# blasif/cocons

Hardware: AMD Instinct MI355X
Metric: -2loglik evals/sec (dense cov_rns + Cholesky/solve/log-det, fp64) at n=10000 (higher is better)
Workload: dtype f64

## Files before the change

cocons_amd/csrc/chol.hip:

```cpp
#include <hip/hip_runtime.h>
#include <limits.h>
#include <stdlib.h>
#include <string.h>
#include <algorithm>
#include <atomic>
#include <vector>
#include "kernels.h"

namespace cocons {

typedef double d4 __attribute__((ext_vector_type(4)));

#define MFMA64(a, b, c) __builtin_amdgcn_mfma_f64_16x16x4f64((a), (b), (c), 0, 0, 0)
#define MFMA64_NEGA(a, b, c) __builtin_amdgcn_mfma_f64_16x16x4f64((a), (b), (c), 0, 0, 1)
#define LDS_T __attribute__((address_space(3)))

__device__ __forceinline__ void blk_mma(d4 &acc, const d4 &P, const d4 &Q)
{
    acc = MFMA64(Q[0], P[0], acc);
    acc = MFMA64(Q[1], P[1], acc);
    acc = MFMA64(Q[2], P[2], acc);
    acc = MFMA64(Q[3], P[3], acc);
}

// ... 1356 lines not shown

#pragma unroll
        for (int v = 0; v < RPT / 2; ++v) {
            stI[v] = *(const d2 *)(gI + 2 * v);
            stJ[v] = *(const d2 *)(gJ + 2 * v);
        }
#pragma unroll
        for (int v = 0; v < RPT / 2; ++v) {
            *(d2 *)(&sI[0][kc * LDT + rg + 2 * v]) = stI[v];
            *(d2 *)(&sJ[0][kc * LDT + rg + 2 * v]) = stJ[v];
        }
        __syncthreads();

        for (int ch = 0; ch < nch; ++ch) {
            const int cur = ch & 1;
            if (ch + 1 < nch) {
                const double *pI = gI + (size_t)(ch + 1) * KC * a.ldp;
                const double *pJ = gJ + (size_t)(ch + 1) * KC * a.ldp;
#pragma unroll
                for (int v = 0; v < RPT / 2; ++v) {
                    stI[v] = *(const d2 *)(pI + 2 * v);
                    stJ[v] = *(const d2 *)(pJ + 2 * v);
                }
            }
            const double *bI = &sI[cur][ro + (TM / 2) * wi];
            const double *bJ = &sJ[cur][ro + (TM / WY) * wj];
#pragma unroll
            for (int s = 0; s < KC / 4; ++s) {
                double pi_[NB], pj_[NBY];
#pragma unroll
                for (int x = 0; x < NB; ++x) pi_[x] = bI[s * 4 * LDT + 16 * x];
#pragma unroll
                for (int y = 0; y < NBY; ++y) pj_[y] = bJ[s * 4 * LDT + 16 * y];
#pragma unroll
                for (int x = 0; x < NB; ++x)
#pragma unroll
                    for (int y = 0; y < NBY; ++y) acc[x][y] = MFMA64(pj_[y], pi_[x], acc[x][y]);
            }
            if (ch + 1 < nch) {
#pragma unroll
                for (int v = 0; v < RPT / 2; ++v) {
                    *(d2 *)(&sI[cur ^ 1][kc * LDT + rg + 2 * v]) = stI[v];
                    *(d2 *)(&sJ[cur ^ 1][kc * LDT + rg + 2 * v]) = stJ[v];
                }
            }
            __syncthreads();
        }
        unsigned Lnext = 0;
        if (a.queue && t2 == 0)
            Lnext = gridDim.x + __hip_atomic_fetch_add(a.queue, 1u, __ATOMIC_RELAXED, __HIP_MEMORY_SCOPE_AGENT);
        unsigned cve = cvo;
        asm volatile("" : "+v"(cve));
#pragma unroll
        for (int x = 0; x < NB; ++x)
#pragma unroll
            for (int y = 0; y < NBY; ++y) {
                d4 cv;
#pragma unroll
                for (int r = 0; r < 4; ++r) {
                    const double *cp = (const double *)((const char *)(Cb + 16 * x) + (cve + (unsigned)(16 * y + 4 * r) * ldcb));
                    cv[r] = a.c_wt ? load_wt(cp) : *cp;
                }
                cv -= acc[x][y];
                if (wt_wg) {
#pragma unroll
                    for (int r = 0; r < 4; ++r)
                        store_wt((double *)((char *)(Cb + 16 * x) + (cve + (unsigned)(16 * y + 4 * r) * ldcb)), cv[r]);
                } else {
#pragma unroll
                    for (int r = 0; r < 4; ++r)
                        *(double *)((char *)(Cb + 16 * x) + (cve + (unsigned)(16 * y + 4 * r) * ldcb)) = cv[r];
                }
            }
        if (wt_wg) {
            asm volatile("s_waitcnt vmcnt(0)" ::: "memory");
            __syncthreads();
            if (t2 == 0 && sig_wg) signal_add(a.sig + a.sig_tile + sig_Ti);
        }
        if (!a.queue) break;
        if (t2 == 0) *share = Lnext;
        __syncthreads();
        L = (unsigned)__builtin_amdgcn_readfirstlane((int)*share);
        if (L >= a.ntiles) break;
    }
}

struct DagStep {
    unsigned base;
    unsigned near;
    unsigned tpos, nT;
    int H, W;
    int tj0;
    int k0, K;
    int nstrip, two;
    int need;
    int nd_next;
    int split;
    unsigned p2, p3;
};

struct DagArgs {
    double *A; size_t lda;
    double *P;
    const double *Wt;
    const DagStep *steps; int nsteps;
    unsigned ntasks;
    unsigned *queue;
    unsigned *tdone;
    unsigned *pdone; int pstride;
    unsigned *pall;
    double *partbuf;
    unsigned *dcount;
    unsigned *sig;
    unsigned *out, *xr;
    unsigned *abort_word;
    const unsigned *alive;
    unsigned xcc_quota;
    unsigned *hw;
    unsigned long long *trace;
    const unsigned *ftab;
    unsigned xcd_g;
    unsigned *xcnt;
};

constexpr unsigned DAG_XCD_LAG = 64u;
__device__ __forceinline__ unsigned dag_position(unsigned c, unsigned cls, unsigned g)
{
    return ((c >> g) << (g + 3u)) | (cls << g) | (c & ((1u << g) - 1u));
}

__device__ __forceinline__ bool dag_wait(const DagArgs &a, unsigned *word, unsigned need, unsigned code, unsigned L)
{
    const unsigned long long t0 = __builtin_amdgcn_s_memrealtime();
    for (unsigned it = 0;; ++it) {
        const unsigned v = poll_word(word, it);
        if (v >= need) break;
        if (__hip_atomic_load(a.abort_word, __ATOMIC_RELAXED, __HIP_MEMORY_SCOPE_AGENT) != 0u) return false;
        if (it > (unsigned)(ENGINE_TIMEOUT_TICKS / 100ull) ||
            ((it & 1023u) == 1023u && __builtin_amdgcn_s_memrealtime() - t0 > WALL_BACKSTOP_TICKS)) {
            if (__hip_atomic_exchange(a.abort_word, code, __ATOMIC_RELAXED, __HIP_MEMORY_SCOPE_AGENT) == 0u) {
                unsigned *d = a.queue + 8;
                d[0] = L; d[1] = code; d[2] = (unsigned)(word - a.queue); d[3] = need; d[4] = v;
                d[5] = (unsigned)(__builtin_amdgcn_s_memrealtime() - t0);
                d[6] = it;
            }
            return false;
        }
        __builtin_amdgcn_s_sleep(16);
    }
    __builtin_amdgcn_fence(__ATOMIC_ACQUIRE, "wavefront");
    return true;
}

__global__ void __launch_bounds__(256, 8)
dag_kernel(DagArgs a)
{
    constexpr int TM = 64, KC = 4, RING = 4, STG = 2 * KC * TM;
    __shared__ double smem[RING * STG + 2];
    unsigned *share = (unsigned *)&smem[RING * STG];
    const int tid = threadIdx.x;
    const int wave_s = __builtin_amdgcn_readfirstlane(tid >> 6);
    const DagStep *__restrict__ steps = a.steps;
    const unsigned ldab = 8u * (unsigned)a.lda;
    int known = 0;
    const unsigned myx = (hw_where() >> 28) & 7u;
    const bool loyal = ((blockIdx.x >> 3) & 1u) == 0u;
    if (tid == 0) {
        bool take = true;
        if (a.xcc_quota) {
            const unsigned c = __hip_atomic_load(a.alive + 16 + myx, __ATOMIC_RELAXED, __HIP_MEMORY_SCOPE_AGENT);
            if (c) {
                const unsigned less = 7u * (c - 1u);
                const unsigned quota = a.xcc_quota > less + 8u ? a.xcc_quota - less : 8u;
                take = __hip_atomic_fetch_add(a.queue + 16 + myx, 1u, __ATOMIC_RELAXED, __HIP_MEMORY_SCOPE_AGENT) < quota;
            }
        }
        unsigned first = 0xffffffffu;
        if (take) {
            if (a.xcd_g) first = dag_position(__hip_atomic_fetch_add(a.xcnt + 32u * myx, 1u, __ATOMIC_RELAXED, __HIP_MEMORY_SCOPE_AGENT), myx, a.xcd_g);
            else first = __hip_atomic_fetch_add(a.queue, 1u, __ATOMIC_RELAXED, __HIP_MEMORY_SCOPE_AGENT);
        }
        share[1] = first;
        share[2] = 0u;
    }
    __syncthreads();
    unsigned L = (unsigned)__builtin_amdgcn_readfirstlane((int)share[1]);
    __syncthreads();
    if (L >= a.ntasks) return;
    for (;;) {
        int lo = 0, hi = a.nsteps - 1;
        while (lo < hi) {
            const int mid = (lo + hi + 1) >> 1;
            if (steps[mid].base <= L) lo = mid; else hi = mid - 1;
        }
        const int s = lo;
        const DagStep st = steps[s];
        const unsigned q = L - st.base;
        if (a.trace && tid == 0) {
            a.trace[4 * (size_t)L] = __builtin_amdgcn_s_memrealtime();
            if (a.hw) a.hw[2 * (size_t)L] = hw_where();
        }
        const int t = st.tj0 >> 1;
        const unsigned per_u = 2u * (unsigned)st.nstrip, nA = per_u + (unsigned)st.nd_next, perBC = st.two ? per_u : 0u;
        int tkind = -1;
        unsigned tu = 0, qt_u = q;
        if (q >= st.tpos) {
            if (q < st.tpos + nA) { tu = q - st.tpos; tkind = tu < per_u ? 0 : 3; }
            else if (q < st.p2) qt_u = q - nA;
            else if (q < st.p2 + perBC) { tu = q - st.p2; tkind = 1; }
            else if (q < st.p3) qt_u = q - nA - perBC;
            else if (q < st.p3 + perBC) { tu = q - st.p3; tkind = 2; }
            else qt_u = q - nA - 2u * perBC;
        }
        const bool isT = tkind >= 0;
        const double *gIb, *gJb;
        unsigned ldib, ldjb, ldob = ldab;
        int K, i_wt = 0, store_only = 0, strip_task = 0;
        double *Cb;
        const double *pa = nullptr;
        unsigned *w0 = nullptr, *w1 = nullptr, *w2 = nullptr, *we = nullptr, *we2 = nullptr, *dn;
        unsigned n0 = 0, n1 = 0, n2 = 0, ne = 0, dval = 0;
        int sigT = -1;
        int prio = 0;
        if (!isT) {
            const int qt = (int)qt_u;
            int ti, tj;
            if (a.ftab && qt >= (int)st.near) {
                const unsigned e = a.ftab[a.ftab[s] + (unsigned)(qt - (int)st.near)];
                tj = st.tj0 + (int)(e & 0xffffu); ti = st.tj0 + (int)(e >> 16);
            } else {
                int jl = 0, jh = st.W - 1;
                while (jl < jh) {
                    const int mid = (jl + jh + 1) >> 1;
                    if (mid * st.H - mid * (mid - 1) / 2 <= qt) jl = mid; else jh = mid - 1;
                }
                tj = st.tj0 + jl; ti = tj + (qt - (jl * st.H - jl * (jl - 1) / 2));
            }
            const double *Ps = s == 0 ? a.A : a.P;
            gIb = Ps + (size_t)ti * TM + (size_t)st.k0 * a.lda;
            gJb = Ps + (size_t)tj * TM + (size_t)st.k0 * a.lda;
            ldib = ldab; ldjb = ldab; K = st.K;
            Cb = a.A + (size_t)ti * TM + (size_t)tj * TM * a.lda;
            if (s > known) {
                w0 = a.pall + s; n0 = (unsigned)st.H;
                w1 = a.pdone + (size_t)s * a.pstride + (ti - st.tj0); n1 = (unsigned)st.need;
                w2 = a.pdone + (size_t)s * a.pstride + (tj - st.tj0); n2 = (unsigned)st.need;
            }
            we = a.tdone + (ti * (ti + 1) / 2 + tj); ne = (unsigned)s;
            dn = we; dval = (unsigned)s + 1u;
            const int Ti = (ti >> 1) - t, Tj = (tj >> 1) - t;
            if (Ti >= 0 && Ti <= st.two && Tj >= 0 && Tj <= Ti) {
                sigT = t + Ti; prio = 3;
                if (st.split) {
                    const int ta = ti - st.tj0, tb = tj - st.tj0, dd = ta * (ta + 1) / 2 + tb;
                    gIb += (size_t)TILE * a.lda; gJb += (size_t)TILE * a.lda; K = TILE;
                    pa = a.partbuf + ((size_t)(s & 1) * 16 + dd) * (TM * TM);
                    we2 = a.dcount + (size_t)s * 16 + dd;
                }
            }
        } else {
            const int per = 2 * st.nstrip;
            const size_t c_t = (size_t)t * TILE, c_t1 = c_t + TILE;
            prio = 2;
            const int stage = tkind;
            int strip = 0, h = 0, row64 = 0;
            if (stage != 3) {
                strip = (int)(tu >> 1); h = (int)(tu & 1u);
                row64 = st.tj0 + (st.two ? 4 : 2) + strip;
                strip_task = 1;
            }
            dn = a.pdone + (size_t)(s + 1) * a.pstride + strip;
            if (stage == 3) {
                const int dd = (int)tu - per;
                const int ta = c_tri_ib[dd], tb = dd - ta * (ta + 1) / 2;
                const int tj0n = st.tj0 + 4;
                const size_t k0n = (size_t)(s + 1) * 2 * TILE;
                gIb = a.P + (size_t)(tj0n + ta) * TM + k0n * a.lda; ldib = ldab;
                gJb = a.P + (size_t)(tj0n + tb) * TM + k0n * a.lda; ldjb = ldab;
                K = TILE;
                Cb = a.partbuf + ((size_t)((s + 1) & 1) * 16 + dd) * (TM * TM); store_only = 1; ldob = 8u * TM;
                w0 = a.pdone + (size_t)(s + 1) * a.pstride + ta; n0 = 2u;
                w1 = a.pdone + (size_t)(s + 1) * a.pstride + tb; n1 = 2u;
                dn = a.dcount + (size_t)(s + 1) * 16 + dd;
            } else if (stage == 0) {
                gIb = a.A + (size_t)row64 * TM + c_t * a.lda; ldib = ldab; i_wt = 1;
                gJb = a.Wt + (size_t)t * TILE * TILE + TM * h; ldjb = 8u * TILE;
                K = TM * (h + 1);
                Cb = a.P + (size_t)row64 * TM + (c_t + TM * h) * a.lda; store_only = 1;
                w0 = a.out + t; n0 = 1u;
                w1 = a.tdone + (row64 * (row64 + 1) / 2 + 2 * t); n1 = (unsigned)s + 1u;
                w2 = w1 + 1; n2 = n1;
            } else if (stage == 1) {
                gIb = a.P + (size_t)row64 * TM + c_t * a.lda; ldib = ldab;
                gJb = a.P + (c_t1 + TM * h) + c_t * a.lda; ldjb = ldab;
                K = TILE;
                Cb = a.A + (size_t)row64 * TM + (c_t1 + TM * h) * a.lda;
                w0 = dn; n0 = 2u;
                w1 = a.xr + t; n1 = 1u;
                we = a.tdone + (row64 * (row64 + 1) / 2 + 2 * (t + 1) + h); ne = (unsigned)s + 1u;
            } else {
                gIb = a.A + (size_t)row64 * TM + c_t1 * a.lda; ldib = ldab; i_wt = 1;
                gJb = a.Wt + (size_t)(t + 1) * TILE * TILE + TM * h; ldjb = 8u * TILE;
                K = TM * (h + 1);
                Cb = a.P + (size_t)row64 * TM + (c_t1 + TM * h) * a.lda; store_only = 1;
                w0 = dn; n0 = 4u;
                w1 = a.out + t + 1; n1 = 1u;
            }
        }
        if (prio == 3) __builtin_amdgcn_s_setprio(3);
        else if (prio == 2) __builtin_amdgcn_s_setprio(2);
        else __builtin_amdgcn_s_setprio(0);

        if (w0) {
            if (tid == 0) {
                unsigned ok;
                if (!isT) {
                    if (__hip_atomic_load(w0, __ATOMIC_RELAXED, __HIP_MEMORY_SCOPE_AGENT) >= n0) ok = 2u;
                    else ok = (dag_wait(a, w1, n1, abort_code(0xb00u, (unsigned)s), L) &&
                               dag_wait(a, w2, n2, abort_code(0xc00u, (unsigned)s), L)) ? 1u : 0u;
                } else {
                    bool o = dag_wait(a, w0, n0, abort_code(0xa00u, (unsigned)s), L);
                    if (o && w1) o = dag_wait(a, w1, n1, abort_code(0xb00u, (unsigned)s), L);
                    if (o && w2) o = dag_wait(a, w2, n2, abort_code(0xc00u, (unsigned)s), L);
                    ok = o ? 1u : 0u;
                }
                *share = ok;
            }
            asm volatile("s_waitcnt vmcnt(0)" ::: "memory");
            __syncthreads();
            const unsigned ok = (unsigned)__builtin_amdgcn_readfirstlane((int)*share);
            __syncthreads();
            if (!ok) return;
            if (ok == 2u) known = s;
        }

        if (a.trace && tid == 0) a.trace[4 * (size_t)L + 1] = __builtin_amdgcn_s_memrealtime();
        int lane;
        asm volatile("v_mbcnt_lo_u32_b32 %0, -1, 0\n\tv_mbcnt_hi_u32_b32 %0, -1, %0" : "=v"(lane));
        const int wave = wave_s, t2 = 64 * wave + lane;
        const int wi = wave & 1, wj = wave >> 1;
        const bool opJ = wave >= 2;
        const char *gsrc = opJ ? (const char *)gJb : (const char *)gIb;
        const unsigned ldg = opJ ? ldjb : ldib, cstep = (unsigned)KC * ldg;
        const bool wt = i_wt && !opJ;
        const int sc = (lane >> 5) & 1;
        const char *src = gsrc + ((unsigned)(2 * (wave & 1) + sc) * ldg + 8u * (unsigned)((2 * (lane & 31)) ^ (16 * sc)));
        LDS_T double *ldst = (LDS_T double *)(smem + 128 * wave);
        const int nch = K / KC;
#define DAG_STAGE(slot)                                                                                                     \
        do {                                                                                                                \
            if (wt) __builtin_amdgcn_global_load_lds((const void *)src, (LDS_T void *)(ldst + STG * (slot)), 16, 0, 16);   \
            else __builtin_amdgcn_global_load_lds((const void *)src, (LDS_T void *)(ldst + STG * (slot)), 16, 0, 0);       \
            src += cstep;                                                                                                   \
        } while (0)
        const int kq = lane >> 4, kodd = kq & 1, rl = (lane & 15) + TM * kq;
        const int aI0 = rl + (TM / 2) * wi + 16 * kodd, aI1 = rl + (TM / 2) * wi + 16 * (kodd ^ 1);
        const int aJ0 = KC * TM + rl + (TM / 2) * wj + 16 * kodd, aJ1 = KC * TM + rl + (TM / 2) * wj + 16 * (kodd ^ 1);
        d4 acc[2][2];
#pragma unroll
        for (int x = 0; x < 2; ++x)
#pragma unroll
            for (int y = 0; y < 2; ++y) acc[x][y] = (d4){0.0, 0.0, 0.0, 0.0};
        DAG_STAGE(0);
        DAG_STAGE(1);
        DAG_STAGE(2);
        for (int c0 = 0; c0 < nch; c0 += RING) {
#pragma unroll
            for (int r = 0; r < RING; ++r) {
                const int ch = c0 + r;
                if (ch + 2 < nch) asm volatile("s_waitcnt vmcnt(2)" ::: "memory");
                else if (ch + 1 < nch) asm volatile("s_waitcnt vmcnt(1)" ::: "memory");
                else asm volatile("s_waitcnt vmcnt(0)" ::: "memory");
                asm volatile("s_waitcnt lgkmcnt(0)" ::: "memory");
                __builtin_amdgcn_s_barrier();
                asm volatile("" ::: "memory");
                if (ch + RING - 1 < nch) DAG_STAGE((r + RING - 1) % RING);
                const double *bs = smem + STG * r;
                const double p0 = bs[aI0], p1 = bs[aI1];
                const double q0 = bs[aJ0], q1 = bs[aJ1];
                acc[0][0] = MFMA64(q0, p0, acc[0][0]);
                acc[0][1] = MFMA64(q1, p0, acc[0][1]);
                acc[1][0] = MFMA64(q0, p1, acc[1][0]);
                acc[1][1] = MFMA64(q1, p1, acc[1][1]);
            }
        }
#undef DAG_STAGE
        if (t2 == 0) {
            unsigned Ln, c = 0u, cy = 0u, cls = 0u, y = 0u;
            unsigned help = 0u;
            if (a.xcd_g) {
                help = loyal ? 0u : share[2];
                cls = help ? help - 1u : myx;
                y = help ? myx : ((myx + 1u + L % 7u) & 7u);
                c = __hip_atomic_fetch_add(a.xcnt + 32u * cls, 1u, __ATOMIC_RELAXED, __HIP_MEMORY_SCOPE_AGENT);
                cy = __hip_atomic_load(a.xcnt + 32u * y, __ATOMIC_RELAXED, __HIP_MEMORY_SCOPE_AGENT);
                Ln = 0u;
            } else
                Ln = __hip_atomic_fetch_add(a.queue, 1u, __ATOMIC_RELAXED, __HIP_MEMORY_SCOPE_AGENT);
            unsigned ok = 1u;
            if (we) ok = dag_wait(a, we, ne, abort_code(0xd00u, (unsigned)s), L) ? 1u : 0u;
            if (ok && we2) ok = wait_ge<false>(we2, 1u, a.abort_word, abort_code(0xe00u, (unsigned)s)) ? 1u : 0u;
            if (a.xcd_g) {
                Ln = dag_position(c, cls, a.xcd_g);
                if (!help) share[2] = (!loyal && c > cy + DAG_XCD_LAG && dag_position(cy, y, a.xcd_g) < a.ntasks) ? y + 1u : 0u;
                else {
                    share[2] = (c + DAG_XCD_LAG / 2u < cy && dag_position(c + 1u, cls, a.xcd_g) < a.ntasks) ? help : 0u;
                    if (Ln >= a.ntasks) {
                        cls = myx;
                        c = __hip_atomic_fetch_add(a.xcnt + 32u * cls, 1u, __ATOMIC_RELAXED, __HIP_MEMORY_SCOPE_AGENT);
                        Ln = dag_position(c, cls, a.xcd_g);
                    }
                }
                if (Ln >= a.ntasks && cls == myx) {
                    for (unsigned d = 1; d < 8u && Ln >= a.ntasks; ++d) {
                        const unsigned z = (myx + d) & 7u;
                        if (dag_position(__hip_atomic_load(a.xcnt + 32u * z, __ATOMIC_RELAXED, __HIP_MEMORY_SCOPE_AGENT), z, a.xcd_g) < a.ntasks)
                            Ln = dag_position(__hip_atomic_fetch_add(a.xcnt + 32u * z, 1u, __ATOMIC_RELAXED, __HIP_MEMORY_SCOPE_AGENT), z, a.xcd_g);
                    }
                }
            }
            share[0] = ok; share[1] = Ln;
            if (a.trace) a.trace[4 * (size_t)L + 2] = __builtin_amdgcn_s_memrealtime();
        }
        asm volatile("s_waitcnt vmcnt(0)" ::: "memory");
        __syncthreads();
        const unsigned okE = share[0];
        const unsigned Lnext = share[1];
        if (!okE) return;
        double *Cw = (double *)((char *)(Cb + (TM / 2) * wi) + (size_t)((TM / 2) * wj) * ldob);
        unsigned cve = 8u * (unsigned)(lane & 15) + (unsigned)(lane >> 4) * ldob;
        asm volatile("" : "+v"(cve));
#pragma unroll
        for (int x = 0; x < 2; ++x)
#pragma unroll
            for (int y = 0; y < 2; ++y) {
                d4 cv;
                if (store_only) cv = acc[x][y];
                else {
#pragma unroll
                    for (int r = 0; r < 4; ++r)
                        cv[r] = load_wt((const double *)((const char *)(Cw + 16 * x) + (cve + (unsigned)(16 * y + 4 * r) * ldob)));
                    if (pa) {
                        const double *Pw = pa + (TM / 2) * wi + (TM / 2) * wj * TM;
                        int ln;
                        asm volatile("v_mbcnt_lo_u32_b32 %0, -1, 0\n\tv_mbcnt_hi_u32_b32 %0, -1, %0" : "=v"(ln));
                        const unsigned cvp = 8u * (unsigned)(ln & 15) + (unsigned)(ln >> 4) * (8u * TM);
                        d4 pv;
#pragma unroll
                        for (int r = 0; r < 4; ++r)
                            pv[r] = load_wt((const double *)((const char *)(Pw + 16 * x) + (cvp + (unsigned)(16 * y + 4 * r) * (8u * TM))));
                        cv -= pv + acc[x][y];
                    } else cv -= acc[x][y];
                }
#pragma unroll
                for (int r = 0; r < 4; ++r)
                    store_wt((double *)((char *)(Cw + 16 * x) + (cve + (unsigned)(16 * y + 4 * r) * ldob)), cv[r]);
            }
        asm volatile("s_waitcnt vmcnt(0)" ::: "memory");
        __syncthreads();
        if (t2 == 0) {
            if (sigT >= 0) signal_add(a.sig + sigT);
            if (dval) __hip_atomic_fetch_max(dn, dval, __ATOMIC_RELAXED, __HIP_MEMORY_SCOPE_AGENT);
            else if (__hip_atomic_fetch_add(dn, 1u, __ATOMIC_RELAXED, __HIP_MEMORY_SCOPE_AGENT) + 1u == (st.two ? 6u : 2u) && strip_task)
                __hip_atomic_fetch_add(a.pall + s + 1, 1u, __ATOMIC_RELAXED, __HIP_MEMORY_SCOPE_AGENT);
            if (a.trace) {
                a.trace[4 * (size_t)L + 3] = __builtin_amdgcn_s_memrealtime();
                if (a.hw) a.hw[2 * (size_t)L + 1] = hw_where();
            }
        }
        L = (unsigned)__builtin_amdgcn_readfirstlane((int)Lnext);
        if (L >= a.ntasks) break;
    }
}

__device__ __forceinline__ double block_sum(double v, double *red)
{
#pragma unroll
    for (int o = 32; o > 0; o >>= 1) v += __shfl_down(v, o, 64);
    int lane = threadIdx.x & 63, wave = threadIdx.x >> 6;
    if (lane == 0) red[wave] = v;
    __syncthreads();
    double t = 0.0;
    if (threadIdx.x == 0)
        for (int w = 0; w < (int)(blockDim.x >> 6); ++w) t += red[w];
    __syncthreads();
    return t;
}

__global__ void __launch_bounds__(1024)
finalize_kernel(const double *A, size_t lda, int c0, int c1, int n, int row0, int nr, double *out, int skew, int npad,
                const double *A2, int a2_cols)
{
    __shared__ double red[16];
    const int b = blockIdx.x;
    const int hi = c1 < n ? c1 : n;
    double s = 0.0;
    constexpr int U = 4;
    const int step = (int)blockDim.x;
    if (b == nr * nr) {
        for (int c = c0 + (int)threadIdx.x; c < hi; c += U * step) {
            double v[U];
#pragma unroll
            for (int q = 0; q < U; ++q) v[q] = (c + q * step < hi) ? A[band_index(c + q * step, c + q * step, lda, skew, npad)] : 1.0;
#pragma unroll
            for (int q = 0; q < U; ++q) s += log(v[q]);
        }
    } else {
        const int ra = row0 + b / nr, rb = row0 + b % nr;
        for (int c = c0 + (int)threadIdx.x; c < hi; c += U * step) {
            double va[U], vb[U];
#pragma unroll
            for (int q = 0; q < U; ++q) {
                const bool in = c + q * step < hi;
                const int cc = c + q * step;
                int below0 = 2 * TILE * (cc / (2 * TILE) + 1);
                if (npad > 0 && below0 > npad) below0 = npad;
                const bool in2 = A2 && cc >= 2 * TILE && cc < a2_cols;
                const double *Sa = (in2 && ra >= below0) ? A2 : A;
                const double *Sb = (in2 && rb >= below0) ? A2 : A;
                va[q] = in ? Sa[band_index(ra, cc, lda, skew, npad)] : 0.0;
                vb[q] = in ? Sb[band_index(rb, cc, lda, skew, npad)] : 0.0;
            }
#pragma unroll
            for (int q = 0; q < U; ++q) s += va[q] * vb[q];
        }
    }
    s = block_sum(s, red);
    if (threadIdx.x == 0) out[b == nr * nr ? 0 : 1 + b] = s;
}

__global__ void __launch_bounds__(256)
row_reduce_kernel(const double *A, size_t lda, int n, int rowy, int row0, int m,
                  double *scratch, int cchunk, int skew, int npad, const double *A2, int a2_cols)
{
    const int i = blockIdx.x * blockDim.x + threadIdx.x;
    const int cb = blockIdx.y * cchunk;
    const int ce = (cb + cchunk < n) ? cb + cchunk : n;
    if (i >= m) return;
    if (A2 && cb >= 2 * TILE && cb < a2_cols) A = A2;
    double s = 0.0, q = 0.0;
    for (int c = cb; c < ce; ++c) {
        double v = A[band_index(row0 + i, c, lda, skew, npad)];
        double y = A[band_index(rowy, c, lda, skew, npad)];
        s = fma(v, y, s);
        q = fma(v, v, q);
    }
    scratch[((size_t)blockIdx.y * 2 + 0) * m + i] = s;
    scratch[((size_t)blockIdx.y * 2 + 1) * m + i] = q;
}

__global__ void __launch_bounds__(256)
row_reduce_final_kernel(const double *scratch, int m, int nchunks, double *stoch, double *quad)
{
    const int i = blockIdx.x * blockDim.x + threadIdx.x;
    if (i >= m) return;
    double s = 0.0, q = 0.0;
    for (int c = 0; c < nchunks; ++c) {
        s += scratch[((size_t)c * 2 + 0) * m + i];
        q += scratch[((size_t)c * 2 + 1) * m + i];
    }
    stoch[i] = s;
    quad[i] = q;
}

__global__ void __launch_bounds__(256)
trmm_lower_kernel(const double *A, size_t lda, int n, const double *E, int lde, int nsim,
                  const double *trend, double *Y, int ldy)
{
    __shared__ double red[4][8][64];
    const int lane = threadIdx.x & 63, wave = threadIdx.x >> 6;
    const int rb = gridDim.x - 1 - blockIdx.x;
    const int i = rb * 64 + lane;
    const int kend = (rb + 1) * 64 < n ? (rb + 1) * 64 : n;
    for (int s0 = 0; s0 < nsim; s0 += 8) {
        double acc[8] = {0, 0, 0, 0, 0, 0, 0, 0};
        for (int k = wave; k < kend; k += 4) {
            double l = (i < n && k <= i) ? A[(size_t)i + (size_t)k * lda] : 0.0;
#pragma unroll
            for (int s = 0; s < 8; ++s)
                if (s0 + s < nsim) acc[s] = fma(l, E[(size_t)k + (size_t)(s0 + s) * lde], acc[s]);
        }
#pragma unroll
        for (int s = 0; s < 8; ++s) red[wave][s][lane] = acc[s];
        __syncthreads();
        if (wave == 0 && i < n) {
#pragma unroll
            for (int s = 0; s < 8; ++s)
                if (s0 + s < nsim)
                    Y[(size_t)i + (size_t)(s0 + s) * ldy] =
                        ((red[0][s][lane] + red[1][s][lane]) + (red[2][s][lane] + red[3][s][lane])) + trend[i];
        }
        __syncthreads();
    }
}

void launch_trmm_lower(const double *A, size_t lda, int n, const double *E, int lde, int nsim,
                       const double *trend, double *Y, int ldy, hipStream_t s)
{
    if (n <= 0 || nsim <= 0) return;
    hipLaunchKernelGGL(trmm_lower_kernel, dim3((n + 63) / 64), dim3(256), 0, s, A, lda, n, E, lde, nsim, trend, Y, ldy);
}

constexpr int BT_COLS = 64;
constexpr size_t BT_LDS_BYTES = (size_t)TILE * BT_COLS * sizeof(double);

__device__ __forceinline__ int bt_lds_index(int k, int j)
{
    return (((k >> 4) * (BT_COLS / 16) + (j >> 4)) << 8) + ((k & 15) << 4) + ((j ^ k) & 15);
}

__global__ void __launch_bounds__(256)
band_trmm_kernel(const double *A, size_t lda, int skew, int npad, const int *hi, int n, const double *E, int lde,
                 int nsim, const double *trend, double *Y, int ldy)
{
    extern __shared__ double Es[];
    const int I = blockIdx.x, s0 = blockIdx.y * BT_COLS;
    const int lane = threadIdx.x & 63, wave = threadIdx.x >> 6;
    int c0 = 0;
    if (hi) {
        int lo = 0, up = I;
        while (lo < up) {
            const int mid = (lo + up) >> 1;
            if (hi[mid] > I) up = mid; else lo = mid + 1;
        }
// ... 140 lines not shown
        const char *x = getenv("COCONS_ENGINE_LDS");
        if (x && (size_t)atol(x) >= shm) shm = (size_t)atol(x);
    }
    return shm;
}

void launch_potrf_engine(double *A, size_t lda, int t0, int nt, double *dinv, int *info,
                         unsigned *in, unsigned *out, unsigned *xr, unsigned *abort_word, unsigned *alive, hipStream_t s,
                         double *wbuf, double *pbuf, int dag_until, unsigned long long *trace, double *mbox, int in_wait_ms)
{
    EngineArgs e;
    e.A = A; e.lda = lda; e.t0 = t0; e.nt = nt; e.dinv = dinv; e.info = info;
    e.in = in; e.out = out; e.xr = xr; e.abort_word = abort_word; e.alive = alive;
    e.wbuf = wbuf; e.pbuf = pbuf; e.dag_until = dag_until; e.trace = trace;
    e.in_ticks = in_wait_ms > 0 ? 100000ull * (unsigned long long)in_wait_ms : HOST_PACED_TICKS;
    e.mbox = mbox;
    e.partner = mbox ? 8 : 0;
    const int grid = e.partner ? e.partner + 1 : 1;
    const size_t shm = engine_lds_bytes();
    if (wbuf && pbuf) {
        static std::atomic<unsigned long long> attr_done{0};
        set_dynamic_lds_once((const void *)potrf_engine_kernel<true>, shm, attr_done);
        hipLaunchKernelGGL(potrf_engine_kernel<true>, dim3(grid), dim3(512), shm, s, e);
    } else {
        static std::atomic<unsigned long long> attr_done{0};
        set_dynamic_lds_once((const void *)potrf_engine_kernel<false>, shm, attr_done);
        hipLaunchKernelGGL(potrf_engine_kernel<false>, dim3(grid), dim3(512), shm, s, e);
    }
}

void launch_trsm_tile(double *A, size_t lda, int c0, int r0, int r1, const double *dinv, hipStream_t s,
                      unsigned *wait_word, unsigned *abort_word, int band_r1, int ext_r0, int own_world, int own_rank,
                      int own_group)
{
    int nb1 = ((band_r1 >= 0 ? band_r1 : r1) - r0) / 64, nb2 = band_r1 >= 0 ? (r1 - ext_r0) / 64 : 0;
    if (nb1 < 0) nb1 = 0;
    if (nb2 < 0) nb2 = 0;
    if (nb1 + nb2 <= 0) return;
    hipLaunchKernelGGL(trsm_tile_kernel, dim3(nb1 + nb2), dim3(256), 0, s, A, lda, c0, r0, dinv, wait_word, abort_word,
                       nb1, ext_r0, own_world, own_rank, own_group < 1 ? 1 : own_group);
}

void launch_potrf_follow(double *A, size_t lda, int c0, int r0, int r1, double *dinv, int *info, double *mbox,
                         unsigned *abort_word, hipStream_t s, int band_r1, int ext_r0)
{
    int nb1 = ((band_r1 >= 0 ? band_r1 : r1) - r0) / 64, nb2 = band_r1 >= 0 ? (r1 - ext_r0) / 64 : 0;
    if (nb1 < 0) nb1 = 0;
    if (nb2 < 0) nb2 = 0;
    const int nstrips = nb1 + nb2;
    static std::atomic<unsigned long long> attr_done{0};
    const size_t shm = 76 * 1024;
    set_dynamic_lds_once((const void *)potrf_follow_kernel, shm, attr_done);
    hipLaunchKernelGGL(potrf_follow_kernel, dim3(1 + (nstrips + 1) / 2), dim3(512), shm, s, A, lda, c0, dinv, info, mbox, r0, nb1,
                       ext_r0, nstrips, abort_word);
}

void launch_panel_pair(double *A, size_t lda, int c0, int r0, int r1, unsigned *xr, unsigned *abort_word, hipStream_t s,
                       const double *mb0, const double *mb1, double *smb, int ndiag, unsigned *sig, int sig_tile, double *xmb)
{
    const int nb = (r1 - r0) / 64;
    if (nb <= 0) return;
    const bool split = xmb != nullptr;
    const bool diag = smb && ndiag > 0 && nb >= (ndiag == 10 ? 4 : 2);
    hipLaunchKernelGGL(panel_pair_kernel, dim3((split ? 2 * nb : nb) + (diag ? ndiag : 0)), dim3(256), 0, s, A, lda, c0, r0,
                       xr, abort_word, mb0, mb1, diag ? smb : nullptr, nb, diag ? (ndiag == 10 ? 4 : 2) : 0, sig, sig_tile, xmb);
}

static int upd_waves = -1;
static long long upd_w8_max_tiles = -1;
void set_update_waves(int nw) { upd_waves = nw == 8 ? 8 : 4; }
void set_update_w8_max_tiles(int ntiles) { upd_w8_max_tiles = ntiles < 0 ? 0 : ntiles; }
static int upd_c_wt = 0;
void set_update_c_wt(int on) { upd_c_wt = on ? 1 : 0; }

void launch_update_from(double *A, size_t lda, const double *P, size_t ldp, int K,
                        int ti0, int ti1, int tj0, int tj1, bool lower_only, hipStream_t s,
                        int ptiles, int world, int rank, unsigned *sig, int sig_tile,
                        unsigned *wait_word, unsigned *abort_word, unsigned *queue, int band_hi, int ext0,
                        int skew, int kblk, int trim64, const int *pmap, int skip_lo, int skip_hi)
{
    const bool band = band_hi >= 0;
    const int rows_band = (band ? band_hi : ti1) - ti0, rows_ext = band ? ti1 - ext0 : 0;
    if (rows_band + rows_ext <= 0 || rows_band < 0 || rows_ext < 0 || tj1 <= tj0 || K <= 0) return;
    trim64 = trim64 ? 1 : 0;
    const int rows64 = 2 * (rows_band + rows_ext) - trim64;
    if (rows64 <= 0) return;
    if (upd_waves < 0) { const char *e = getenv("COCONS_UPD_WAVES"); set_update_waves(e ? atoi(e) : 8); }
    if (upd_w8_max_tiles < 0) { const char *e = getenv("COCONS_UPD_W8_MAX_TILES"); set_update_w8_max_tiles(e ? atoi(e) : 3500); }
    bool use_w8 = false;
    UpdArgs a;
    a.queue = nullptr; a.ntiles = 0;
    a.skew = skew; a.kblk = kblk; a.c_wt = upd_c_wt;
    a.Hb = 2 * rows_band; a.ext0 = 2 * ext0;
    a.C = A; a.ldc = lda; a.P = P; a.ldp = ldp; a.K = K;
    a.lower_only = lower_only ? 1 : 0;
    a.ptiles = ptiles < 1 ? 1 : ptiles; a.world = world; a.rank = rank; a.pmap = pmap; a.skip_lo = skip_lo; a.skip_hi = skip_hi;
    a.sig = sig; a.sig_tile = sig_tile;
    a.wait_word = wait_word; a.abort_word = abort_word;
    a.H = 0; a.W = 0;
    a.ti0 = 2 * ti0; a.tj0 = 2 * tj0;
    dim3 grid(rows64, 2 * (tj1 - tj0));
    if (lower_only) {
        if (ti0 != tj0) { a.lower_only = 0; }
        else {
            const long long H = rows64, W = 2LL * (tj1 - tj0);
            a.H = (int)H; a.W = (int)W;
            const long long total = W * H - W * (W - 1) / 2;
            static int slots = 0;
            if (!slots) {
                int dev = 0, cus = 256;
                hipGetDevice(&dev);
                hipDeviceGetAttribute(&cus, hipDeviceAttributeMultiprocessorCount, dev);
                slots = 8 * cus;
            }
            grid = dim3((unsigned)total, 1);
            if (queue && world == 1) {
                const bool w8 = upd_waves == 8 && K >= 2 * TILE && !skew &&
                                (upd_w8_max_tiles == 0 || total <= upd_w8_max_tiles);
                use_w8 = w8;
                const int cap = w8 ? slots / 2 - 4 : slots - 8;
                if (total > cap + (w8 ? 4 : 8)) {
                    a.queue = queue; a.ntiles = (unsigned)total;
                    grid = dim3((unsigned)cap, 1);
                }
            }
        }
    }
    const bool trailing = (K > TILE) && world == 1;
    if (trailing && use_w8 && a.lower_only) hipLaunchKernelGGL((update_kernel<64, 16, 0, 8>), grid, dim3(512), 0, s, a);
    else if (trailing) hipLaunchKernelGGL((update_kernel<64, 8, 0>), grid, dim3(256), 0, s, a);
    else hipLaunchKernelGGL((update_kernel<64, 8, 1>), grid, dim3(256), 0, s, a);
}

__global__ void __launch_bounds__(256)
pack_rows_kernel(const double *A, size_t lda, int col0, int ncols, double *dst, size_t ldp, const int *pmap, int ti_lo,
                 long long slot_lo, long long slot_hi)
{
    const int ti = ti_lo + (int)blockIdx.x;
    const long long off = pmap[ti];
    if (off < slot_lo || off >= slot_hi) return;
    const int rho = threadIdx.x & 63, cq = threadIdx.x >> 6;
    for (int c = 4 * (int)blockIdx.y + cq; c < ncols; c += 4 * (int)gridDim.y)
        dst[off + rho + (size_t)c * ldp] = A[(size_t)(64 * ti + rho) + (size_t)(col0 + c) * lda];
}

void launch_pack_rows(const double *A, size_t lda, int col0, int ncols, double *dst, size_t ldp, const int *pmap, int ti_lo,
                      int ti_hi, long long slot_lo, long long slot_hi, hipStream_t s)
{
    if (ti_hi <= ti_lo || ncols <= 0) return;
    hipLaunchKernelGGL(pack_rows_kernel, dim3(ti_hi - ti_lo, 8), dim3(256), 0, s, A, lda, col0, ncols, dst, ldp, pmap, ti_lo,
                       slot_lo, slot_hi);
}

static void dag_build_far_table(const std::vector<DagStepHost> &steps, std::vector<unsigned> &tab, int xcd_g, int bw, int bh)
{
    tab.assign(steps.size(), 0u);
    for (size_t s = 0; s < steps.size(); ++s) {
        const DagStepHost &st = steps[s];
        tab[s] = (unsigned)tab.size();
        const int nc = std::min(st.W, st.two ? 4 : 2);
        std::vector<std::vector<unsigned>> blocks;
        if (bw <= 0) {
            blocks.emplace_back();
            for (int jl = nc; jl < st.W; ++jl)
                for (int il = jl; il < st.H; ++il) blocks.back().push_back((unsigned)il << 16 | (unsigned)jl);
        } else {
            for (int c0 = nc; c0 < st.W; c0 += bw) {
                const int c1 = std::min(c0 + bw, st.W);
                for (int r0 = c0; r0 < st.H; r0 += bh) {
                    const int r1 = std::min(r0 + bh, st.H);
                    std::vector<unsigned> b;
                    for (int il = r0; il < r1; ++il)
                        for (int jl = c0; jl < c1 && jl <= il; ++jl) b.push_back((unsigned)il << 16 | (unsigned)jl);
                    if (!b.empty()) blocks.push_back(std::move(b));
                }
            }
        }
        const long long ntile = (long long)st.W * st.H - (long long)st.W * (st.W - 1) / 2;
        const long long nfar = ntile - st.near;
        const unsigned nA = 2u * (unsigned)st.nstrip + (unsigned)st.nd_next, perBC = st.two ? 2u * (unsigned)st.nstrip : 0u;
        const bool panels = st.nT > 0;
        size_t next_block = 0;
        size_t cur[8], pos_in[8];
        for (int x = 0; x < 8; ++x) { cur[x] = (size_t)-1; pos_in[x] = 0; }
        std::vector<size_t> taken_back(blocks.size(), 0);
        long long q = 0;
        const unsigned total = (unsigned)ntile + st.nT;
        for (unsigned pos = 0; pos < total && q < ntile; ++pos) {
            if (panels && ((pos >= st.tpos && pos < st.tpos + nA) || (pos >= st.p2 && pos < st.p2 + perBC) ||
                           (pos >= st.p3 && pos < st.p3 + perBC)))
                continue;
            const long long qt = q++;
            if (qt < (long long)st.near) continue;
            const int x = xcd_g > 0 ? (int)(((st.base + pos) >> xcd_g) & 7u) : 0;
            unsigned tile = 0;
            bool got = false;
            while (!got) {
                if (cur[x] != (size_t)-1 && pos_in[x] + taken_back[cur[x]] < blocks[cur[x]].size()) {
                    tile = blocks[cur[x]][pos_in[x]++];
                    got = true;
                } else if (next_block < blocks.size()) {
                    cur[x] = next_block++; pos_in[x] = 0;
                } else {
                    size_t best = (size_t)-1, left = 0;
                    for (int y = 0; y < 8; ++y)
                        if (cur[y] != (size_t)-1) {
                            const size_t l = blocks[cur[y]].size() - pos_in[y] - taken_back[cur[y]];
                            if (l > left) { left = l; best = cur[y]; }
                        }
                    if (best == (size_t)-1) break;
                    tile = blocks[best][blocks[best].size() - 1 - taken_back[best]++];
                    got = true;
                }
            }
            tab.push_back(tile);
        }
        (void)nfar;
    }
}

unsigned dag_build_steps(int nt, int mt, int trim64, int kskip, int lead, int min_tiles, std::vector<DagStepHost> &out,
                         int lead2, int lead3, std::vector<unsigned> *ftab, int xcd_g, int bw, int bh)
{
    out.clear();
    if (ftab) ftab->clear();
    unsigned base = 0;
    int prev_two = 1;
    for (int k = 0; k + 2 < nt; k += 2) {
        const int t = k + 2;
        {
            const long long H0 = 2LL * (mt - t) - (trim64 ? 1 : 0), W0 = 2LL * (nt - t);
            if (W0 * H0 - W0 * (W0 - 1) / 2 < min_tiles) break;
        }
        DagStepHost st;
        st.tj0 = 2 * t;
        st.H = 2 * (mt - t) - (trim64 ? 1 : 0);
        st.W = 2 * (nt - t);
        st.two = t + 1 < nt ? 1 : 0;
        const long long tiles = (long long)st.W * st.H - (long long)st.W * (st.W - 1) / 2;
        const int nc = std::min(st.W, st.two ? 4 : 2);
        st.near = (unsigned)(nc * st.H - nc * (nc - 1) / 2);
        st.nstrip = std::max(0, st.H - (st.two ? 4 : 2));
        st.nT = (unsigned)(st.nstrip * (st.two ? 6 : 2));
        st.k0 = k * TILE + (k == 0 ? kskip : 0);
        st.K = 2 * TILE - (k == 0 ? kskip : 0);
        st.need = prev_two ? 6 : 2;
        st.nd_next = 0; st.split = 0;
        st.tpos = 0; st.p2 = 0; st.p3 = 0;
        st.base = 0;
        prev_two = st.two;
        (void)tiles;
        out.push_back(st);
    }
    if (!out.empty()) {
        DagStepHost &l = out.back();
        l.nT = 0; l.nstrip = 0;
    }
    for (size_t s = 0; s + 1 < out.size(); ++s)
        if (out[s].nstrip > 0 && out[s].two) {
            out[s].nd_next = out[s + 1].two ? 10 : 3;
            out[s + 1].split = 1;
        }
    for (auto &st : out) {
        const long long ntile = (long long)st.W * st.H - (long long)st.W * (st.W - 1) / 2;
        st.nT += (unsigned)st.nd_next;
        const long long nA = 2LL * st.nstrip + st.nd_next;
        const long long perBC = st.two ? 2LL * st.nstrip : 0;
        const long long far = ntile - st.near;
        st.tpos = st.near + (unsigned)std::min<long long>(far, lead);
        st.base = base;
        base += (unsigned)ntile + st.nT;
        long long rem = ntile - (long long)st.tpos;
        if (st.nT == 0) { st.p2 = st.p3 = st.tpos; continue; }
        const long long d2 = std::min<long long>(rem, perBC ? lead2 : 0);
        rem -= d2;
        const long long d3 = std::min<long long>(rem, perBC ? lead3 : 0);
        st.p2 = (unsigned)(st.tpos + nA + d2);
        st.p3 = (unsigned)(st.p2 + perBC + d3);
    }
    if (ftab) dag_build_far_table(out, *ftab, xcd_g, bw, bh);
    return base;
}

void launch_dag(double *A, size_t lda, double *P, const double *Wt, const DagStepHost *dsteps, int nsteps, unsigned ntasks,
                unsigned *queue, unsigned *tdone, unsigned *pdone, int pstride, unsigned *pall, double *partbuf, unsigned *dcount,
                unsigned *sig, unsigned *out, unsigned *xr, unsigned *abort_word, hipStream_t s, unsigned long long *trace,
                const unsigned *alive, int xcc_quota, unsigned *hw, const unsigned *ftab, int xcd_g, unsigned *xcnt)
{
    static_assert(sizeof(DagStepHost) == sizeof(DagStep), "host and device step records");
    if (nsteps <= 0 || ntasks == 0) return;
    DagArgs a;
    a.A = A; a.lda = lda; a.P = P; a.Wt = Wt;
    a.steps = (const DagStep *)dsteps; a.nsteps = nsteps; a.ntasks = ntasks;
    a.queue = queue; a.tdone = tdone; a.pdone = pdone; a.pstride = pstride; a.pall = pall;
    a.partbuf = partbuf; a.dcount = dcount;
    a.sig = sig; a.out = out; a.xr = xr; a.abort_word = abort_word; a.trace = trace; a.hw = trace ? hw : nullptr;
    static int slots = 0;
    if (!slots) {
        int dev = 0, cus = 256;
        hipGetDevice(&dev);
        hipDeviceGetAttribute(&cus, hipDeviceAttributeMultiprocessorCount, dev);
        slots = 8 * cus;
    }
    const unsigned cap = (unsigned)(slots - 8);
    a.alive = alive; a.xcc_quota = (alive && xcc_quota > 0) ? (unsigned)xcc_quota : 0u;
    a.ftab = ftab; a.xcd_g = (ftab && xcnt && xcd_g > 0) ? (unsigned)xcd_g : 0u;
    a.xcnt = xcnt;
    hipLaunchKernelGGL(dag_kernel, dim3(ntasks < cap ? ntasks : cap), dim3(256), 0, s, a);
}

void launch_update(double *A, size_t lda, int k0, int K, int ti0, int ti1, int tj0, int tj1,
                   bool lower_only, hipStream_t s, unsigned *sig, int sig_tile,
                   unsigned *wait_word, unsigned *abort_word, unsigned *queue, int band_hi, int ext0,
                   int skew, int trim64, int skip_lo, int skip_hi)
{
    launch_update_from(A, lda, A + (size_t)k0 * lda, lda, K, ti0, ti1, tj0, tj1, lower_only, s, 1, 1, 0, sig, sig_tile,
                       wait_word, abort_word, queue, band_hi, ext0, skew, k0 / TILE, trim64, nullptr, skip_lo, skip_hi);
}

void launch_finalize_cols(const double *A, size_t lda, int c0, int c1, int n, int row0, int nr,
                          double *out, hipStream_t s)
{
    hipLaunchKernelGGL(finalize_kernel, dim3(nr * nr + 1), dim3(1024), 0, s, A, lda, c0, c1, n, row0, nr, out, 0, 0,
                       (const double *)nullptr, 0);
}

void launch_finalize(const double *A, size_t lda, int n, int row0, int nr, double *out, hipStream_t s, int skew, int npad,
                     const double *A2, int a2_cols)
{
    hipLaunchKernelGGL(finalize_kernel, dim3(nr * nr + 1), dim3(1024), 0, s, A, lda, 0, n, n, row0, nr, out, skew, npad,
                       skew ? (const double *)nullptr : A2, a2_cols);
}

size_t row_reduce_scratch_doubles(int n, int m)
{
    return (size_t)2 * (size_t)m * (size_t)((n + 255) / 256);
}

void launch_row_reduce(const double *A, size_t lda, int n, int rowy, int row0, int m,
                       double *stoch, double *quad, double *scratch, hipStream_t s, int skew, int npad,
                       const double *A2, int a2_cols)
{
    if (m <= 0) return;
    const int cchunk = 2 * TILE, nchunks = (n + cchunk - 1) / cchunk;
    hipLaunchKernelGGL(row_reduce_kernel, dim3((m + 255) / 256, nchunks), dim3(256), 0, s,
                       A, lda, n, rowy, row0, m, scratch, cchunk, skew, npad, skew ? (const double *)nullptr : A2, a2_cols);
    hipLaunchKernelGGL(row_reduce_final_kernel, dim3((m + 255) / 256), dim3(256), 0, s,
                       scratch, m, nchunks, stoch, quad);
}



__device__ __forceinline__ void krige_tile_ij(int t, int &I, int &J)
{
    int i = (int)((sqrt(8.0 * t + 1.0) - 1.0) * 0.5);
    while ((i + 1) * (i + 2) / 2 <= t) ++i;
    while (i * (i + 1) / 2 > t) --i;
    I = i; J = t - i * (i + 1) / 2;
}

__global__ void __launch_bounds__(256)
krige_pack_kernel(const double *A, size_t lda, double *Lp)
{
    int I, J;
    krige_tile_ij((int)blockIdx.x, I, J);
    const double *src = A + (size_t)I * TILE + (size_t)J * TILE * lda;
    double *dst = Lp + (size_t)blockIdx.x * TILE * TILE;
    for (int e = threadIdx.x; e < TILE * TILE; e += 256) {
        const int r = e & (TILE - 1), c = e >> 7;
        const double v = src[(size_t)r + (size_t)c * lda];
        dst[e] = (I == J && r < c) ? 0.0 : v;
    }
}

__global__ void __launch_bounds__(256)
krige_qprep_kernel(const double *A, size_t lda, int rowy, int c_lo, int c_hi, double *Qp, double *w)
{
    const int J = blockIdx.x, tid = threadIdx.x;
    if (tid < TILE) {
        const int c = J * TILE + tid;
        w[c] = (c >= c_lo && c < c_hi) ? A[(size_t)rowy + (size_t)c * lda] : 0.0;
    }
    for (int e = tid; e < 8 * 256; e += 256) {
        const int jb = e >> 8, s = (e >> 6) & 3, lane = e & 63;
        const int m = lane & 15, k = lane >> 4, c = m & 3;
        double q = 0.0;
        if ((m >> 2) == s && k <= c) {
            const double *L = A + (size_t)(J * TILE + 16 * jb + 4 * s) * (1 + lda);
            const double l10 = L[1], l20 = L[2], l30 = L[3], l21 = L[2 + lda], l31 = L[3 + lda], l32 = L[3 + 2 * lda];
            const double r0 = 1.0 / L[0], r1 = 1.0 / L[1 + lda], r2 = 1.0 / L[2 + 2 * lda], r3 = 1.0 / L[3 + 3 * lda];
            const double m00 = r0, m11 = r1, m22 = r2, m33 = r3;
            const double m10 = -(l10 * m00) * r1;
            const double m21 = -(l21 * m11) * r2;
            const double m32 = -(l32 * m22) * r3;
            const double m20 = -fma(l21, m10, l20 * m00) * r2;
            const double m31 = -fma(l32, m21, l31 * m11) * r3;
            const double m30 = -fma(l32, m20, fma(l31, m10, l30 * m00)) * r3;
            q = sel_lower4(c, k, m00, m10, m11, m20, m21, m22, m30, m31, m32, m33);
        }
        Qp[(size_t)J * 2048 + e] = q;
    }
}

__global__ void __launch_bounds__(256)
krige_diag_kernel(const double *Lp, const double *Qp, const double *w, double *C, size_t ldc, int J, int c_lo, int c_hi,
                  double *stoch, double *quad)
{
    __shared__ double SL[36 * 256];
    __shared__ double QS[8 * 256];
    const int tid = threadIdx.x, lane = tid & 63, wave = tid >> 6;
    fetch_factor_tile<false>(Lp + (size_t)(J * (J + 1) / 2 + J) * TILE * TILE, TILE, 0, Qp + (size_t)J * 2048, SL, QS, tid);
    const int rs = 64 * (int)blockIdx.x + 16 * wave, c0 = J * TILE;
    d4 B[8];
#pragma unroll
    for (int j = 0; j < 8; ++j) {
        B[j] = glb_blk(C, ldc, rs, c0 + 16 * j, lane);
#pragma unroll
        for (int r = 0; r < 4; ++r) {
            const int c = c0 + 16 * j + 4 * r + (lane >> 4);
            if (c < c_lo || c >= c_hi) B[j][r] = 0.0;
        }
    }
    __syncthreads();
#pragma unroll
    for (int j = 0; j < 8; ++j) {
        d4 L = lds_blk(SL + (j * (j + 1) / 2 + j) * 256, lane);
        double Q[4];
#pragma unroll
        for (int s = 0; s < 4; ++s) Q[s] = QS[j * 256 + s * 64 + lane];
        trsm16(B[j], L, Q);
        d4 NX = -B[j];
#pragma unroll
        for (int jj = j + 1; jj < 8; ++jj) {
// ... 91 lines not shown
```

Before: 124.2.

## Cache DAG step table in LDS, prefetch far-tile entries and next-task atomics

Copies the first 48 step records into shared memory and replaces the per-task binary search over global step records with a check that the task is still in the current step, falling back to a search over the LDS table. The far-tile table is re-indexed by global task id so the next task's tile entry can be loaded early and carried across iterations. The queue fetch-add, the cross-XCD counter load and the epilogue wait-word load are issued two chunks before the K loop ends, which overlaps their latency with the MFMA work. The cost is more LDS per workgroup (asserted to stay within eight workgroups per CU), a larger far table, and dequeueing slightly earlier.

```diff
diff --git a/cocons_amd/csrc/chol.hip b/cocons_amd/csrc/chol.hip
--- a/cocons_amd/csrc/chol.hip
+++ b/cocons_amd/csrc/chol.hip
@@ -1532,15 +1532,31 @@
     return true;
 }
 
+constexpr int DAG_TAB_STEPS = 48;
+static_assert(sizeof(DagStep) == 64, "a step record is 16 words in the on-chip table");
+
+__device__ __forceinline__ unsigned dag_step_word(LDS_T const unsigned *stab, const DagStep *steps, int i, int w)
+{
+    unsigned v;
+    if (i < DAG_TAB_STEPS) v = stab[16 * i + w];
+    else v = ((const unsigned *)steps)[16 * (size_t)i + w];
+    return (unsigned)__builtin_amdgcn_readfirstlane((int)v);
+}
+
 __global__ void __launch_bounds__(256, 8)
 dag_kernel(DagArgs a)
 {
     constexpr int TM = 64, KC = 4, RING = 4, STG = 2 * KC * TM;
-    __shared__ double smem[RING * STG + 2];
+    constexpr int CTRL = 8;
+    __shared__ double smem[RING * STG + CTRL / 2 + DAG_TAB_STEPS * 8];
+    static_assert(sizeof(smem) <= 20480, "eight workgroups per CU");
     unsigned *share = (unsigned *)&smem[RING * STG];
+    LDS_T unsigned *stab = (LDS_T unsigned *)(share + CTRL);
     const int tid = threadIdx.x;
     const int wave_s = __builtin_amdgcn_readfirstlane(tid >> 6);
     const DagStep *__restrict__ steps = a.steps;
+    for (int i = tid; i < 16 * (a.nsteps < DAG_TAB_STEPS ? a.nsteps : DAG_TAB_STEPS); i += 256)
+        stab[i] = ((const unsigned *)steps)[i];
     const unsigned ldab = 8u * (unsigned)a.lda;
     int known = 0;
     const unsigned myx = (hw_where() >> 28) & 7u;
@@ -1567,19 +1583,42 @@
     unsigned L = (unsigned)__builtin_amdgcn_readfirstlane((int)share[1]);
     __syncthreads();
     if (L >= a.ntasks) return;
+    int s = 0;
+    unsigned help_s = 0u;
+    unsigned e_far = a.ftab ? a.ftab[L] : 0u;
     for (;;) {
-        int lo = 0, hi = a.nsteps - 1;
-        while (lo < hi) {
-            const int mid = (lo + hi + 1) >> 1;
-            if (steps[mid].base <= L) lo = mid; else hi = mid - 1;
-        }
-        const int s = lo;
-        const DagStep st = steps[s];
-        const unsigned q = L - st.base;
         if (a.trace && tid == 0) {
             a.trace[4 * (size_t)L] = __builtin_amdgcn_s_memrealtime();
             if (a.hw) a.hw[2 * (size_t)L] = hw_where();
         }
+        {
+            const unsigned b0 = dag_step_word(stab, steps, s, 0);
+            const unsigned b1 = s + 1 < a.nsteps ? dag_step_word(stab, steps, s + 1, 0) : a.ntasks;
+            if (L - b0 >= b1 - b0) {
+                int lo = 0, hi = a.nsteps - 1;
+                while (lo < hi) {
+                    const int mid = (lo + hi + 1) >> 1;
+                    if (dag_step_word(stab, steps, mid, 0) <= L) lo = mid; else hi = mid - 1;
+                }
+                s = lo;
+            } else if (a.trace && tid == 0)
+                __hip_atomic_fetch_add(a.queue + 41, 1u, __ATOMIC_RELAXED, __HIP_MEMORY_SCOPE_AGENT);
+        }
+        DagStep st;
+        {
+            unsigned w[16];
+            if (s < DAG_TAB_STEPS) {
+#pragma unroll
+                for (int i = 0; i < 16; ++i) w[i] = stab[16 * s + i];
+            } else {
+#pragma unroll
+                for (int i = 0; i < 16; ++i) w[i] = ((const unsigned *)steps)[16 * (size_t)s + i];
+            }
+#pragma unroll
+            for (int i = 0; i < 16; ++i) w[i] = (unsigned)__builtin_amdgcn_readfirstlane((int)w[i]);
+            __builtin_memcpy(&st, w, sizeof st);
+        }
+        const unsigned q = L - st.base;
         const int t = st.tj0 >> 1;
         const unsigned per_u = 2u * (unsigned)st.nstrip, nA = per_u + (unsigned)st.nd_next, perBC = st.two ? per_u : 0u;
         int tkind = -1;
@@ -1606,7 +1645,7 @@
             const int qt = (int)qt_u;
             int ti, tj;
             if (a.ftab && qt >= (int)st.near) {
-                const unsigned e = a.ftab[a.ftab[s] + (unsigned)(qt - (int)st.near)];
+                const unsigned e = (unsigned)__builtin_amdgcn_readfirstlane((int)e_far);
                 tj = st.tj0 + (int)(e & 0xffffu); ti = st.tj0 + (int)(e >> 16);
             } else {
                 int jl = 0, jh = st.W - 1;
@@ -1744,6 +1783,7 @@
         DAG_STAGE(0);
         DAG_STAGE(1);
         DAG_STAGE(2);
+        unsigned dr_c = 0u, dr_cy = 0u, dr_we = 0u;
         for (int c0 = 0; c0 < nch; c0 += RING) {
 #pragma unroll
             for (int r = 0; r < RING; ++r) {
@@ -1755,6 +1795,14 @@
                 __builtin_amdgcn_s_barrier();
                 asm volatile("" ::: "memory");
                 if (ch + RING - 1 < nch) DAG_STAGE((r + RING - 1) % RING);
+                if (r == RING - 2 && ch + 2 == nch && t2 == 0) {
+                    unsigned coff = a.xcd_g ? 32u * (help_s ? help_s - 1u : myx) : 0u;
+                    asm volatile("" : "+v"(coff));
+                    dr_c = __hip_atomic_fetch_add((a.xcd_g ? a.xcnt : a.queue) + coff, 1u, __ATOMIC_RELAXED, __HIP_MEMORY_SCOPE_AGENT);
+                    if (a.xcd_g)
+                        dr_cy = __hip_atomic_load(a.xcnt + 32u * (help_s ? myx : ((myx + 1u + L % 7u) & 7u)), __ATOMIC_RELAXED, __HIP_MEMORY_SCOPE_AGENT);
+                    if (we) dr_we = __hip_atomic_load(we, __ATOMIC_RELAXED, __HIP_MEMORY_SCOPE_AGENT);
+                }
                 const double *bs = smem + STG * r;
                 const double p0 = bs[aI0], p1 = bs[aI1];
                 const double q0 = bs[aJ0], q1 = bs[aJ1];
@@ -1766,19 +1814,15 @@
         }
 #undef DAG_STAGE
         if (t2 == 0) {
-            unsigned Ln, c = 0u, cy = 0u, cls = 0u, y = 0u;
+            unsigned Ln = dr_c, c = dr_c, cy = dr_cy, cls = 0u, y = 0u;
             unsigned help = 0u;
             if (a.xcd_g) {
-                help = loyal ? 0u : share[2];
+                help = help_s;
                 cls = help ? help - 1u : myx;
                 y = help ? myx : ((myx + 1u + L % 7u) & 7u);
-                c = __hip_atomic_fetch_add(a.xcnt + 32u * cls, 1u, __ATOMIC_RELAXED, __HIP_MEMORY_SCOPE_AGENT);
-                cy = __hip_atomic_load(a.xcnt + 32u * y, __ATOMIC_RELAXED, __HIP_MEMORY_SCOPE_AGENT);
-                Ln = 0u;
-            } else
-                Ln = __hip_atomic_fetch_add(a.queue, 1u, __ATOMIC_RELAXED, __HIP_MEMORY_SCOPE_AGENT);
+            }
             unsigned ok = 1u;
-            if (we) ok = dag_wait(a, we, ne, abort_code(0xd00u, (unsigned)s), L) ? 1u : 0u;
+            if (we && dr_we < ne) ok = dag_wait(a, we, ne, abort_code(0xd00u, (unsigned)s), L) ? 1u : 0u;
             if (ok && we2) ok = wait_ge<false>(we2, 1u, a.abort_word, abort_code(0xe00u, (unsigned)s)) ? 1u : 0u;
             if (a.xcd_g) {
                 Ln = dag_position(c, cls, a.xcd_g);
@@ -1806,7 +1850,10 @@
         __syncthreads();
         const unsigned okE = share[0];
         const unsigned Lnext = share[1];
+        help_s = (unsigned)__builtin_amdgcn_readfirstlane((int)share[2]);
         if (!okE) return;
+        unsigned e_next = 0u;
+        if (a.ftab && Lnext < a.ntasks) e_next = a.ftab[(unsigned)__builtin_amdgcn_readfirstlane((int)Lnext)];
         double *Cw = (double *)((char *)(Cb + (TM / 2) * wi) + (size_t)((TM / 2) * wj) * ldob);
         unsigned cve = 8u * (unsigned)(lane & 15) + (unsigned)(lane >> 4) * ldob;
         asm volatile("" : "+v"(cve));
@@ -1850,6 +1897,7 @@
         }
         L = (unsigned)__builtin_amdgcn_readfirstlane((int)Lnext);
         if (L >= a.ntasks) break;
+        e_far = e_next;
     }
 }
 
@@ -2296,12 +2344,12 @@
                        slot_lo, slot_hi);
 }
 
-static void dag_build_far_table(const std::vector<DagStepHost> &steps, std::vector<unsigned> &tab, int xcd_g, int bw, int bh)
-{
-    tab.assign(steps.size(), 0u);
+static void dag_build_far_table(const std::vector<DagStepHost> &steps, unsigned ntasks, std::vector<unsigned> &tab, int xcd_g,
+                                int bw, int bh)
+{
+    tab.assign(ntasks, 0u);
     for (size_t s = 0; s < steps.size(); ++s) {
         const DagStepHost &st = steps[s];
-        tab[s] = (unsigned)tab.size();
         const int nc = std::min(st.W, st.two ? 4 : 2);
         std::vector<std::vector<unsigned>> blocks;
         if (bw <= 0) {
@@ -2357,7 +2405,7 @@
                     got = true;
                 }
             }
-            tab.push_back(tile);
+            tab[st.base + pos] = tile;
         }
         (void)nfar;
     }
@@ -2422,7 +2470,7 @@
         st.p2 = (unsigned)(st.tpos + nA + d2);
         st.p3 = (unsigned)(st.p2 + perBC + d3);
     }
-    if (ftab) dag_build_far_table(out, *ftab, xcd_g, bw, bh);
+    if (ftab) dag_build_far_table(out, base, *ftab, xcd_g, bw, bh);
     return base;
 }
 
```

Result: no change. 123.3, median of 2 (-0.7%).
